# voletiv/mcvd-pytorch

Hardware: NVIDIA H100
Metric: frames/sec @100 DDPM steps, SMMNIST 64x64 (higher is better)
Workload: dtype f32 (fp16 hi/lo split on wgmma, fp32 accumulate)

## Files before the change

include/mcvd_b200.h:

```cpp
#ifndef MCVD_B200_H
#define MCVD_B200_H

#include <stdint.h>

#ifdef __cplusplus
extern "C" {
#endif

#define MCVD_ABI_VERSION 5

enum {
  MCVD_OP_NCHW_TO_NHWC = 1,
  MCVD_OP_NHWC_TO_NCHW = 2,
  MCVD_OP_TIMESTEP_EMBED = 3,
  MCVD_OP_LINEAR = 4,
  MCVD_OP_GN_PARTIAL = 5,
  MCVD_OP_GN_FINALIZE = 6,
  MCVD_OP_APPLY = 7,
  MCVD_OP_CONV_SIMT = 8,
  MCVD_OP_ATTENTION = 9,
  MCVD_OP_RESIZE_NEAREST = 10,
  MCVD_OP_DIFFUSION_UPDATE = 11,
  MCVD_OP_CONV_UMMA = 12,
  MCVD_OP_CONV_SMALLN = 13,
  MCVD_OP_COPY = 14,
  MCVD_OP_ATTENTION_UMMA = 15,
  MCVD_OP_CONV_UMMA2 = 16,
  MCVD_OP_FRAME_METRICS = 17,
  MCVD_OP_NOISE = 18,
  MCVD_OP_LPIPS_PREP = 19,
  MCVD_OP_CONV_RELU = 20,
  MCVD_OP_LPIPS_LAYER = 21,
  MCVD_OP_I3D_PREP = 22,
  MCVD_OP_CONV3D = 23,
  MCVD_OP_MAXPOOL3D = 24,
  MCVD_OP_I3D_HEAD = 25,
  MCVD_OP__COUNT
};

#define MCVD_F_ACT_IN   (1 << 0)
#define MCVD_F_ACT_OUT  (1 << 1)
#define MCVD_F_UP       (1 << 2)
#define MCVD_F_DOWN     (1 << 3)
#define MCVD_F_FILM     (1 << 4)
#define MCVD_F_CLIP     (1 << 5)
#define MCVD_F_PHILOX   (1 << 6)
#define MCVD_F_ROUND    (1 << 7)
#define MCVD_F_GAMMA    (1 << 8)
#define MCVD_F_POOL     (1 << 9)

typedef struct McvdOp {
  int32_t kind;
  int32_t flags;
  int32_t B, H, W;
  int32_t C0, C1;
  int32_t Cout;
  int32_t i0, i1, i2, i3;
  float f0, f1, f2, f3, f4, f5, f6, f7;
  const void* src0;
  const void* src1;
  const void* w;
  const void* bias;
  const void* aux0;
  const void* aux1;
  const void* aux2;
  void* dst;
  void* dst2;
  const void* src2;
  const void* src3;
  int32_t C2, C3;
  int32_t i4, i5, i6, i7;
} McvdOp;

int mcvd_abi_version(void);
int mcvd_sizeof_op(void);
const char* mcvd_last_error(void);
int mcvd_device_arch(void);

int mcvd_run_program(const McvdOp* ops, int n, void* stream);

int mcvd_validate_program(const McvdOp* ops, int n);

int mcvd_count_launches(const McvdOp* ops, int n);

long long mcvd_umma_pack_weights(const float* w_taps, int taps, int Cin, int Cout, int n_tile, int k_block,
                                 void* out, int scale_log2, void* stream);
int mcvd_umma_kblock(int C0, int C1);
int mcvd_umma2_plan(int H, int W, int ks, int C0, int C1, int C2, int C3, int n_tile, int stats);
int mcvd_umma2_plan_info(int H, int W, int ks, int C0, int C1, int C2, int C3, int n_tile, int stats, int* out);
long long mcvd_umma2_stats_bytes(int B, int H, int W, int ks, int Cout);
long long mcvd_umma2_pack_weights(const float* w_taps, int taps, int Cin, int Cout, int n_tile, int k_block,
                                  void* out, int scale_log2, int stage_off, int per_unit, void* stream);
long long mcvd_attention_scratch_bytes(int B, int T, int C);

#ifdef __cplusplus
}
#endif
#endif
```

mcvd_b200/csrc/api.cu:

```cuda
#include <stdarg.h>
#include <string.h>

#include "mcvd_common.cuh"

namespace mcvd {

static thread_local char g_err[512] = {0};

void set_error(const char* fmt, ...) {
  va_list ap;
  va_start(ap, fmt);
  vsnprintf(g_err, sizeof(g_err), fmt, ap);
  va_end(ap);
}

static int dispatch(const McvdOp& op, cudaStream_t s) {
  switch (op.kind) {
    case MCVD_OP_NCHW_TO_NHWC: return launch_nchw_to_nhwc(op, s);
    case MCVD_OP_NHWC_TO_NCHW: return launch_nhwc_to_nchw(op, s);
    case MCVD_OP_TIMESTEP_EMBED: return launch_timestep_embed(op, s);
    case MCVD_OP_LINEAR: return launch_linear(op, s);
    case MCVD_OP_GN_PARTIAL: return launch_gn_partial(op, s);
    case MCVD_OP_GN_FINALIZE: return launch_gn_finalize(op, s);
    case MCVD_OP_APPLY: return launch_apply(op, s);
    case MCVD_OP_CONV_SIMT: return launch_conv_simt(op, s);
    case MCVD_OP_ATTENTION: return launch_attention(op, s);
    case MCVD_OP_RESIZE_NEAREST: return launch_resize_nearest(op, s);
    case MCVD_OP_DIFFUSION_UPDATE: return launch_diffusion_update(op, s);
    case MCVD_OP_CONV_UMMA: return launch_conv_umma(op, s);
    case MCVD_OP_CONV_UMMA2: return launch_conv_umma2(op, s);
    case MCVD_OP_CONV_SMALLN: return launch_conv_smalln(op, s);
    case MCVD_OP_COPY: return launch_copy(op, s);
    case MCVD_OP_ATTENTION_UMMA: return launch_attention_umma(op, s);
    case MCVD_OP_FRAME_METRICS: return launch_frame_metrics(op, s);
    case MCVD_OP_NOISE: return launch_noise(op, s);
    case MCVD_OP_LPIPS_PREP: return launch_lpips_prep(op, s);
    case MCVD_OP_CONV_RELU: return launch_conv_relu(op, s);
    case MCVD_OP_LPIPS_LAYER: return launch_lpips_layer(op, s);
    case MCVD_OP_I3D_PREP: return launch_i3d_prep(op, s);
    case MCVD_OP_CONV3D: return launch_conv3d(op, s);
    case MCVD_OP_MAXPOOL3D: return launch_maxpool3d(op, s);
    case MCVD_OP_I3D_HEAD: return launch_i3d_head(op, s);
    default: break;
  }
  set_error("unknown op kind %d", op.kind);
  return -1;
}

static int validate_one(const McvdOp& op, int idx) {
  if (op.kind <= 0 || op.kind >= MCVD_OP__COUNT) {
    set_error("op %d: unknown kind %d", idx, op.kind);
    return -1;
  }
  if (op.B <= 0) {
    set_error("op %d (kind %d): batch %d", idx, op.kind, op.B);
    return -1;
  }
  const bool spatial = op.kind != MCVD_OP_TIMESTEP_EMBED && op.kind != MCVD_OP_LINEAR && op.kind != MCVD_OP_COPY;
  if (spatial && (op.H <= 0 || op.W <= 0)) {
    set_error("op %d (kind %d): spatial size %dx%d", idx, op.kind, op.H, op.W);
    return -1;
  }
  if (!op.dst || (!op.src0 && op.kind != MCVD_OP_NOISE)) {
    set_error("op %d (kind %d): null src0/dst", idx, op.kind);
    return -1;
  }
  if (op.C1 > 0 && !op.src1 && op.kind != MCVD_OP_DIFFUSION_UPDATE) {
    set_error("op %d (kind %d): C1=%d but src1 is null", idx, op.kind, op.C1);
    return -1;
  }
  auto misaligned = [](const void* p) { return p && (reinterpret_cast<uintptr_t>(p) & 15) != 0; };
  if (misaligned(op.src0) || misaligned(op.src1) || misaligned(op.dst) || misaligned(op.w) || misaligned(op.aux0) ||
      misaligned(op.aux1) || misaligned(op.aux2)) {
    set_error("op %d (kind %d): pointers must be 16-byte aligned", idx, op.kind);
    return -1;
  }
  switch (op.kind) {
    case MCVD_OP_APPLY:
      if (op.C0 % 4 || op.C1 % 4) {
        set_error("op %d APPLY: channels (%d,%d) not multiples of 4", idx, op.C0, op.C1);
        return -1;
      }
      break;
    case MCVD_OP_CONV_SIMT:
    case MCVD_OP_CONV_UMMA:
    case MCVD_OP_CONV_UMMA2:
      if (!op.w || (op.i0 != 1 && op.i0 != 3)) {
        set_error("op %d CONV: null weights or kernel size %d", idx, op.i0);
        return -1;
      }
      break;
    case MCVD_OP_ATTENTION:
    case MCVD_OP_ATTENTION_UMMA:
      if (op.i0 * op.i1 != op.C0) {
        set_error("op %d ATTENTION: heads %d x dim %d != %d", idx, op.i0, op.i1, op.C0);
        return -1;
      }
      if (op.kind == MCVD_OP_ATTENTION_UMMA && (!op.dst2 || (reinterpret_cast<uintptr_t>(op.dst2) & 15))) {
        set_error("op %d ATTENTION_UMMA: dst2 (operand-image scratch) is null or not 16-byte aligned", idx);
        return -1;
      }
      break;
    case MCVD_OP_DIFFUSION_UPDATE:
    case MCVD_OP_NOISE:
      if (op.flags & MCVD_F_GAMMA) {
        if (op.kind == MCVD_OP_DIFFUSION_UPDATE && !(op.flags & MCVD_F_PHILOX)) {
          set_error("op %d DIFFUSION_UPDATE: MCVD_F_GAMMA needs MCVD_F_PHILOX", idx);
          return -1;
        }
        if (const char* why = gamma_params_error(op)) {
          set_error("op %d (kind %d): %s", idx, op.kind, why);
          return -1;
        }
      }
      break;
    case MCVD_OP_LPIPS_PREP:
      if (!op.src1 || !op.w) {
        set_error("op %d LPIPS_PREP: null real frames or resize table", idx);
        return -1;
      }
      if (op.C0 != 1 && op.C0 != 3) {
        set_error("op %d LPIPS_PREP: %d channels per frame (1 or 3)", idx, op.C0);
        return -1;
      }
      if (op.H != 128 || op.W != 128) {
        set_error("op %d LPIPS_PREP: output side %dx%d (must be 128x128)", idx, op.H, op.W);
        return -1;
      }
      if (op.i0 < 1 || op.i1 < 1 || op.i2 < 1 || 2LL * op.B * op.i0 > 65535) {
        set_error("op %d LPIPS_PREP: %d frames of side %d, %d taps, batch %d", idx, op.i0, op.i1, op.i2, op.B);
        return -1;
      }
      break;
    case MCVD_OP_CONV_RELU:
      if (const char* why = conv_relu_error(op)) {
        set_error("op %d CONV_RELU: %s", idx, why);
        return -1;
      }
      if (misaligned(op.bias)) {
        set_error("op %d CONV_RELU: bias must be 16-byte aligned", idx);
        return -1;
      }
      break;
    case MCVD_OP_LPIPS_LAYER:
      if (!op.src1 || !op.w || op.C0 < 1) {
        set_error("op %d LPIPS_LAYER: null real features or lin weights, or %d channels", idx, op.C0);
        return -1;
      }
      break;
    case MCVD_OP_I3D_PREP:
    case MCVD_OP_CONV3D:
    case MCVD_OP_MAXPOOL3D:
    case MCVD_OP_I3D_HEAD: {
      const char* why = op.kind == MCVD_OP_I3D_PREP ? i3d_prep_error(op)
                        : op.kind == MCVD_OP_CONV3D  ? conv3d_error(op)
                        : op.kind == MCVD_OP_MAXPOOL3D ? maxpool3d_error(op)
                                                       : i3d_head_error(op);
      static const char* const names[] = {"I3D_PREP", "CONV3D", "MAXPOOL3D", "I3D_HEAD"};
      if (why) {
        set_error("op %d %s: %s", idx, names[op.kind - MCVD_OP_I3D_PREP], why);
        return -1;
      }
      if (misaligned(op.bias)) {
        set_error("op %d %s: bias must be 16-byte aligned", idx, names[op.kind - MCVD_OP_I3D_PREP]);
        return -1;
      }
      break;
    }
    default: break;
  }
  return 0;
}

}

extern "C" {

int mcvd_abi_version(void) { return MCVD_ABI_VERSION; }
int mcvd_sizeof_op(void) { return (int)sizeof(McvdOp); }
const char* mcvd_last_error(void) { return mcvd::g_err; }

int mcvd_device_arch(void) {
  int dev = 0;
  if (cudaGetDevice(&dev) != cudaSuccess) {
    cudaGetLastError();
    mcvd::set_error("no CUDA device");
    return -1;
  }
  cudaDeviceProp p;
  if (cudaGetDeviceProperties(&p, dev) != cudaSuccess) {
    cudaGetLastError();
    mcvd::set_error("cudaGetDeviceProperties failed");
    return -1;
  }
  return p.major * 10 + p.minor;
}

int mcvd_validate_program(const McvdOp* ops, int n) {
  if (!ops || n < 0) {
    mcvd::set_error("null program");
    return -1;
  }
  for (int i = 0; i < n; ++i) {
    int r = mcvd::validate_one(ops[i], i);
    if (r) return r;
  }
  return 0;
}

int mcvd_count_launches(const McvdOp* ops, int n) {
  if (!ops || n < 0) return -1;
  int total = 0;
  for (int i = 0; i < n; ++i) total += (ops[i].kind == MCVD_OP_ATTENTION_UMMA) ? 2 : 1;
  return total;
}

int mcvd_run_program(const McvdOp* ops, int n, void* stream) {
  if (!ops || n < 0) {
    mcvd::set_error("null program");
    return -1;
  }
  cudaStream_t s = reinterpret_cast<cudaStream_t>(stream);
  for (int i = 0; i < n; ++i) {
    int r = mcvd::dispatch(ops[i], s);
    if (r) {
      char tmp[400];
      strncpy(tmp, mcvd::g_err, sizeof(tmp) - 1);
      tmp[sizeof(tmp) - 1] = 0;
      mcvd::set_error("op %d (kind %d): %s", i, ops[i].kind, tmp);
      return r;
    }
  }
  return 0;
}

}
```

mcvd_b200/csrc/attention_umma.cu:

```cuda
#include "mcvd_common.cuh"
#include "umma_ptx.cuh"

namespace mcvd {

namespace {

using namespace ptx;

constexpr int QT = 128;
constexpr int ATT_THREADS = 288;
constexpr int SPLIT_THREADS = 256;

struct AttnArgs {
  const float* qkv;
  float* out;
  uint8_t* img;
  long long k_off, v_off;
  int T, C, KT, nkt, nqt, nst;
  float scale;
};

__device__ __forceinline__ void split8(const float v[8], uint4& hv, uint4& lv) {
  uint32_t hw[4], lw[4];
#pragma unroll
  for (int e = 0; e < 4; ++e) split2(v[2 * e], v[2 * e + 1], hw[e], lw[e]);
  hv = make_uint4(hw[0], hw[1], hw[2], hw[3]);
  lv = make_uint4(lw[0], lw[1], lw[2], lw[3]);
}

template <int D>
__device__ __forceinline__ void stage_rows(uint8_t* hi, uint8_t* lo, const float* src, long long stride, int rows,
                                           int valid_rows, int tid, int nthreads) {
  constexpr int U = 6;
  const int units = (D / 8) * rows;
  for (int u0 = tid; u0 < units; u0 += nthreads * U) {
    float4 va[U], vb[U];
#pragma unroll
    for (int i = 0; i < U; ++i) {
      const int u = u0 + i * nthreads;
      const int c8 = u / rows, r = u - c8 * rows;
      va[i] = vb[i] = make_float4(0.f, 0.f, 0.f, 0.f);
      if (u < units && r < valid_rows) {
        const float4* p = reinterpret_cast<const float4*>(src + (long long)r * stride + c8 * 8);
        va[i] = __ldg(p);
        vb[i] = __ldg(p + 1);
      }
    }
#pragma unroll
    for (int i = 0; i < U; ++i) {
      const int u = u0 + i * nthreads;
      if (u < units) {
        const int c8 = u / rows, r = u - c8 * rows;
        const float v[8] = {va[i].x, va[i].y, va[i].z, va[i].w, vb[i].x, vb[i].y, vb[i].z, vb[i].w};
        uint4 hv, lv;
        split8(v, hv, lv);
        const size_t off = ((size_t)c8 * rows + r) * 16;
        *reinterpret_cast<uint4*>(hi + off) = hv;
        *reinterpret_cast<uint4*>(lo + off) = lv;
      }
    }
  }
}

template <int D>
__device__ __forceinline__ void stage_v(uint8_t* vh, uint8_t* vl, const float* vsrc, long long stride, int KT, int tid,
                                        int nthreads) {
  constexpr int C4 = D / 4;
  const int vunits = (KT / 8) * C4;
  for (int u0 = tid; u0 < vunits; u0 += 2 * nthreads) {
    float4 ld[2][8];
#pragma unroll
    for (int i = 0; i < 2; ++i) {
      const int u = u0 + i * nthreads;
      const int kc = u / C4, c4 = u - kc * C4;
#pragma unroll
      for (int e = 0; e < 8; ++e)
        ld[i][e] = (u < vunits) ? __ldg(reinterpret_cast<const float4*>(vsrc + (long long)(kc * 8 + e) * stride) + c4)
                                : make_float4(0.f, 0.f, 0.f, 0.f);
    }
#pragma unroll
    for (int i = 0; i < 2; ++i) {
      const int u = u0 + i * nthreads;
      if (u < vunits) {
        const int kc = u / C4, c4 = u - kc * C4;
        const float r0[8] = {ld[i][0].x, ld[i][1].x, ld[i][2].x, ld[i][3].x, ld[i][4].x, ld[i][5].x, ld[i][6].x, ld[i][7].x};
        const float r1[8] = {ld[i][0].y, ld[i][1].y, ld[i][2].y, ld[i][3].y, ld[i][4].y, ld[i][5].y, ld[i][6].y, ld[i][7].y};
        const float r2[8] = {ld[i][0].z, ld[i][1].z, ld[i][2].z, ld[i][3].z, ld[i][4].z, ld[i][5].z, ld[i][6].z, ld[i][7].z};
        const float r3[8] = {ld[i][0].w, ld[i][1].w, ld[i][2].w, ld[i][3].w, ld[i][4].w, ld[i][5].w, ld[i][6].w, ld[i][7].w};
        uint4 hv, lv;
        const size_t off = ((size_t)kc * D + c4 * 4) * 16;
        split8(r0, hv, lv); *reinterpret_cast<uint4*>(vh + off) = hv;      *reinterpret_cast<uint4*>(vl + off) = lv;
        split8(r1, hv, lv); *reinterpret_cast<uint4*>(vh + off + 16) = hv; *reinterpret_cast<uint4*>(vl + off + 16) = lv;
        split8(r2, hv, lv); *reinterpret_cast<uint4*>(vh + off + 32) = hv; *reinterpret_cast<uint4*>(vl + off + 32) = lv;
        split8(r3, hv, lv); *reinterpret_cast<uint4*>(vh + off + 48) = hv; *reinterpret_cast<uint4*>(vl + off + 48) = lv;
      }
    }
  }
}

template <int D> __host__ __device__ constexpr int kt_max() { return D <= 96 ? 128 : (D <= 128 ? 64 : 32); }

template <int D> __host__ __device__ constexpr long long q_image_bytes() { return 2LL * (D / 8) * QT * 16; }
template <int D> __host__ __device__ inline long long kv_image_bytes(int KT) { return 2LL * (D / 8) * KT * 16; }

template <int D>
__global__ void __launch_bounds__(SPLIT_THREADS) k_attn_presplit(const AttnArgs a) {
  const int x = blockIdx.x, h = blockIdx.y, b = blockIdx.z, heads = gridDim.y;
  const int C3 = 3 * a.C, KT = a.KT;
  const float* base = a.qkv + (long long)b * a.T * C3 + h * D;
  const long long bh = (long long)b * heads + h;
  if (x < a.nqt) {
    uint8_t* dst = a.img + (bh * a.nqt + x) * q_image_bytes<D>();
    const int q0 = x * QT;
    stage_rows<D>(dst, dst + q_image_bytes<D>() / 2, base + (long long)q0 * C3, C3, QT, min(QT, a.T - q0), threadIdx.x,
                  SPLIT_THREADS);
  } else if (x < a.nqt + a.nkt) {
    const int kt = x - a.nqt;
    uint8_t* dst = a.img + a.k_off + (bh * a.nkt + kt) * kv_image_bytes<D>(KT);
    stage_rows<D>(dst, dst + kv_image_bytes<D>(KT) / 2, base + a.C + (long long)kt * KT * C3, C3, KT, KT, threadIdx.x,
                  SPLIT_THREADS);
  } else {
    const int kt = x - a.nqt - a.nkt;
    uint8_t* dst = a.img + a.v_off + (bh * a.nkt + kt) * kv_image_bytes<D>(KT);
    stage_v<D>(dst, dst + kv_image_bytes<D>(KT) / 2, base + 2 * a.C + (long long)kt * KT * C3, C3, KT, threadIdx.x,
               SPLIT_THREADS);
  }
}

template <int D, int KT>
__global__ void __launch_bounds__(ATT_THREADS, 1) k_attention_umma(const AttnArgs a) {
  extern __shared__ __align__(1024) uint8_t smem_raw[];
  constexpr int NQ = QT / 64;
  const int NST = a.nst;
  const uint32_t q_bytes = (uint32_t)q_image_bytes<D>(), kv_bytes = (uint32_t)kv_image_bytes<D>(KT);
  uint8_t* qimg = smem_raw;
  uint8_t* kimg = qimg + q_bytes;
  uint8_t* vimg = kimg + (size_t)NST * kv_bytes;
  uint64_t* bars = reinterpret_cast<uint64_t*>(vimg + (size_t)NST * kv_bytes);
  const uint32_t bar0 = smem_u32(bars);
  const uint32_t Q_FULL = bar0;
  auto K_FULL = [&](int i) { return bar0 + 8u * (1 + i); };
  auto V_FULL = [&](int i) { return bar0 + 8u * (3 + i); };
  auto K_EMPTY = [&](int i) { return bar0 + 8u * (5 + i); };
  auto V_EMPTY = [&](int i) { return bar0 + 8u * (7 + i); };

  const int tid = threadIdx.x, warp = tid >> 5, lane = tid & 31;
  const int q0 = blockIdx.x * QT, h = blockIdx.y, b = blockIdx.z;
  const long long bh = (long long)b * gridDim.y + h;

  if (tid == 0) {
    mbar_init(Q_FULL, 1);
    for (int i = 0; i < 2; ++i) {
      mbar_init(K_FULL(i), 1); mbar_init(V_FULL(i), 1);
      mbar_init(K_EMPTY(i), 4 * NQ); mbar_init(V_EMPTY(i), 4 * NQ);
    }
    fence_barrier_init();
  }
  __syncthreads();

  if (warp == 4 * NQ) {
    if (elect_one()) {
      mbar_arrive_expect_tx(Q_FULL, q_bytes);
      bulk_g2s(smem_u32(qimg), a.img + (bh * a.nqt + blockIdx.x) * q_image_bytes<D>(), q_bytes, Q_FULL);
      for (int kt = 0; kt < a.nkt; ++kt) {
        const int st = kt % NST;
        const uint32_t ph = ((kt / NST) & 1) ^ 1;
        const long long off = (bh * a.nkt + kt) * kv_image_bytes<D>(KT);
        mbar_wait(K_EMPTY(st), ph);
        mbar_arrive_expect_tx(K_FULL(st), kv_bytes);
        bulk_g2s(smem_u32(kimg + (size_t)st * kv_bytes), a.img + a.k_off + off, kv_bytes, K_FULL(st));
        mbar_wait(V_EMPTY(st), ph);
        mbar_arrive_expect_tx(V_FULL(st), kv_bytes);
        bulk_g2s(smem_u32(vimg + (size_t)st * kv_bytes), a.img + a.v_off + off, kv_bytes, V_FULL(st));
      }
    }
    __syncwarp();
    return;
  }

  const int wg = warp >> 2, wq = warp & 3;
  const int r0 = 64 * wg + 16 * wq + (lane >> 2);
  const int cq = 2 * (lane & 3);
  const uint64_t q_desc = make_desc(smem_u32(qimg) + 64u * 16u * wg, QT * 16, 128);
  const uint32_t q_lo16 = q_bytes / 32;
  const uint32_t kv_lo16 = kv_bytes / 32;
  float m[2] = {-INFINITY, -INFINITY}, l[2] = {0.f, 0.f};
  float o[D / 2];
#pragma unroll
  for (int i = 0; i < D / 2; ++i) o[i] = 0.f;
  mbar_wait(Q_FULL, 0);
  for (int kt = 0; kt < a.nkt; ++kt) {
    const int st = kt % NST;
    const uint32_t ph = (kt / NST) & 1;
    float sacc[KT / 2];
    const uint64_t k_desc = make_desc(smem_u32(kimg + (size_t)st * kv_bytes), KT * 16, 128);
    mbar_wait(K_FULL(st), ph);
    wgmma_fence();
#pragma unroll
    for (int s = 0; s < D / 16; ++s) {
      const uint64_t qh = desc_add(q_desc, 2u * s * QT), ql = desc_add(qh, q_lo16);
      const uint64_t kh = desc_add(k_desc, 2u * s * KT), kl = desc_add(kh, kv_lo16);
      wgmma_ss<KT>(sacc, qh, kh, s);
      wgmma_ss<KT>(sacc, ql, kh, 1);
      wgmma_ss<KT>(sacc, qh, kl, 1);
    }
    wgmma_commit();
    wgmma_wait<0>();
#pragma unroll
    for (int i = 0; i < KT / 2; ++i) reg_fence(sacc[i]);
    if (lane == 0) mbar_arrive(K_EMPTY(st));
    float alpha[2];
#pragma unroll
    for (int i = 0; i < 2; ++i) {
      float mx = -INFINITY;
#pragma unroll
      for (int j = 0; j < KT / 8; ++j)
        mx = fmaxf(mx, fmaxf(sacc[4 * j + 2 * i], sacc[4 * j + 2 * i + 1]));
      mx = fmaxf(mx, __shfl_xor_sync(0xffffffffu, mx, 1));
      mx = fmaxf(mx, __shfl_xor_sync(0xffffffffu, mx, 2));
      const float mn = fmaxf(m[i], mx * a.scale);
      alpha[i] = expf(m[i] - mn);
      m[i] = mn;
      float sum = 0.f;
#pragma unroll
      for (int j = 0; j < KT / 8; ++j) {
#pragma unroll
        for (int e = 0; e < 2; ++e) {
          const float p = expf(fmaf(sacc[4 * j + 2 * i + e], a.scale, -mn));
          sacc[4 * j + 2 * i + e] = p;
          sum += p;
        }
      }
      l[i] = l[i] * alpha[i] + sum;
    }
#pragma unroll
    for (int j = 0; j < D / 8; ++j) {
      o[4 * j] *= alpha[0]; o[4 * j + 1] *= alpha[0];
      o[4 * j + 2] *= alpha[1]; o[4 * j + 3] *= alpha[1];
    }
    const uint64_t v_desc = make_desc(smem_u32(vimg + (size_t)st * kv_bytes), D * 16, 128);
    mbar_wait(V_FULL(st), ph);
    uint32_t ph4[KT / 16][4], pl4[KT / 16][4];
#pragma unroll
    for (int kk = 0; kk < KT / 16; ++kk)
#pragma unroll
      for (int r = 0; r < 4; ++r) split2(sacc[8 * kk + 2 * r], sacc[8 * kk + 2 * r + 1], ph4[kk][r], pl4[kk][r]);
    wgmma_fence();
#pragma unroll
    for (int kk = 0; kk < KT / 16; ++kk) {
      const uint64_t vh = desc_add(v_desc, 2u * kk * D), vl = desc_add(vh, kv_lo16);
      wgmma_rs<D>(o, ph4[kk], vh);
      wgmma_rs<D>(o, pl4[kk], vh);
      wgmma_rs<D>(o, ph4[kk], vl);
    }
    wgmma_commit();
    wgmma_wait<0>();
#pragma unroll
    for (int i = 0; i < D / 2; ++i) reg_fence(o[i]);
    if (lane == 0) mbar_arrive(V_EMPTY(st));
  }
#pragma unroll
  for (int i = 0; i < 2; ++i) {
    l[i] += __shfl_xor_sync(0xffffffffu, l[i], 1);
    l[i] += __shfl_xor_sync(0xffffffffu, l[i], 2);
  }
#pragma unroll
  for (int i = 0; i < 2; ++i) {
    const int q = q0 + r0 + 8 * i;
    if (q >= a.T) continue;
    const float inv = 1.0f / l[i];
    float* orow = a.out + ((long long)b * a.T + q) * a.C + h * D;
#pragma unroll
    for (int j = 0; j < D / 8; ++j)
      *reinterpret_cast<float2*>(orow + 8 * j + cq) = make_float2(o[4 * j + 2 * i] * inv, o[4 * j + 2 * i + 1] * inv);
  }
}

template <int D, int KT>
int launch_dk(const AttnArgs& a, size_t smem, const McvdOp& op, cudaStream_t s) {
  cudaError_t e = cudaFuncSetAttribute(k_attention_umma<D, KT>, cudaFuncAttributeMaxDynamicSharedMemorySize, (int)smem);
  MCVD_CHECK(e == cudaSuccess, "ATTENTION_UMMA: cudaFuncSetAttribute failed: %s", cudaGetErrorString(e));
  dim3 sgrid(a.nqt + 2 * a.nkt, op.i0, op.B);
  k_attn_presplit<D><<<sgrid, SPLIT_THREADS, 0, s>>>(a);
  MCVD_CUDA_LAUNCH_CHECK("attention presplit");
  dim3 grid(a.nqt, op.i0, op.B);
  k_attention_umma<D, KT><<<grid, ATT_THREADS, smem, s>>>(a);
  MCVD_CUDA_LAUNCH_CHECK("attention_umma");
  return 0;
}

template <int D>
int launch_d(const McvdOp& op, cudaStream_t s) {
  AttnArgs a;
  a.qkv = (const float*)op.src0; a.out = (float*)op.dst;
  a.T = op.H * op.W; a.C = op.C0; a.scale = op.f0;
  a.KT = kt_max<D>();
  if (a.T < a.KT) a.KT = a.T;
  MCVD_CHECK((a.KT == 32 || a.KT == 64 || a.KT == 128) && a.T % a.KT == 0,
             "ATTENTION_UMMA: %d tokens not tileable by the key tile %d", a.T, a.KT);
  a.nkt = a.T / a.KT;
  a.nqt = cdiv(a.T, QT);
  a.img = (uint8_t*)op.dst2;
  const long long bh = (long long)op.B * op.i0;
  a.k_off = bh * a.nqt * q_image_bytes<D>();
  a.v_off = a.k_off + bh * a.nkt * kv_image_bytes<D>(a.KT);
  MCVD_CHECK(op.dst2, "ATTENTION_UMMA: dst2 (operand-image scratch, mcvd_attention_scratch_bytes) is NULL");
  MCVD_CHECK((reinterpret_cast<uintptr_t>(op.dst2) & 15) == 0, "ATTENTION_UMMA: scratch must be 16-byte aligned");
  const size_t q_bytes = (size_t)q_image_bytes<D>(), kv_bytes = (size_t)kv_image_bytes<D>(a.KT);
  a.nst = (q_bytes + 4 * kv_bytes + 128 <= 227 * 1024) ? 2 : 1;
  const size_t smem = q_bytes + 2 * a.nst * kv_bytes + 128;
  MCVD_CHECK(smem <= 227 * 1024, "ATTENTION_UMMA: %zu B of shared memory", smem);
  if (a.KT == 32) return launch_dk<D, 32>(a, smem, op, s);
  if (a.KT == 64) return launch_dk<D, (kt_max<D>() >= 64 ? 64 : 32)>(a, smem, op, s);
  return launch_dk<D, kt_max<D>()>(a, smem, op, s);
}

}

long long attention_umma_scratch_bytes(int B, int T, int C) {
  if (B <= 0 || T <= 0 || C <= 0) return 0;
  return 4LL * B * C * ((long long)cdiv(T, QT) * QT + 2LL * T);
}

int launch_attention_umma(const McvdOp& op, cudaStream_t s) {
  MCVD_CHECK(op.src0 && op.dst, "ATTENTION_UMMA: null pointer");
  MCVD_CHECK(op.i0 * op.i1 == op.C0, "ATTENTION_UMMA: heads %d x dim %d != channels %d", op.i0, op.i1, op.C0);
  switch (op.i1) {
    case 32: return launch_d<32>(op, s);
    case 48: return launch_d<48>(op, s);
    case 64: return launch_d<64>(op, s);
    case 96: return launch_d<96>(op, s);
    case 128: return launch_d<128>(op, s);
    case 192: return launch_d<192>(op, s);
    default: break;
  }
  set_error("ATTENTION_UMMA: head dim %d unsupported (32/48/64/96/128/192)", op.i1);
  return -1;
}

}

extern "C" long long mcvd_attention_scratch_bytes(int B, int T, int C) {
  return mcvd::attention_umma_scratch_bytes(B, T, C);
}
```

mcvd_b200/lib.py:

```python
from __future__ import annotations

import ctypes as C
import os
import threading

from . import build as _build

OP_NCHW_TO_NHWC = 1
OP_NHWC_TO_NCHW = 2
OP_TIMESTEP_EMBED = 3
OP_LINEAR = 4
OP_GN_PARTIAL = 5
OP_GN_FINALIZE = 6
OP_APPLY = 7
OP_CONV_SIMT = 8
OP_ATTENTION = 9
OP_RESIZE_NEAREST = 10
OP_DIFFUSION_UPDATE = 11
OP_CONV_UMMA = 12
OP_CONV_SMALLN = 13
OP_COPY = 14
OP_ATTENTION_UMMA = 15
OP_CONV_UMMA2 = 16
OP_FRAME_METRICS = 17
OP_NOISE = 18
OP_LPIPS_PREP = 19
OP_CONV_RELU = 20
OP_LPIPS_LAYER = 21
OP_I3D_PREP = 22
OP_CONV3D = 23
OP_MAXPOOL3D = 24
OP_I3D_HEAD = 25

F_ACT_IN = 1 << 0
F_ACT_OUT = 1 << 1
F_UP = 1 << 2
F_DOWN = 1 << 3
F_FILM = 1 << 4
F_CLIP = 1 << 5
F_PHILOX = 1 << 6
F_ROUND = 1 << 7
F_GAMMA = 1 << 8
F_POOL = 1 << 9

ABI_VERSION = 5

EXPORTS = ["mcvd_abi_version", "mcvd_sizeof_op", "mcvd_last_error", "mcvd_device_arch", "mcvd_run_program",
           "mcvd_validate_program", "mcvd_count_launches", "mcvd_umma_pack_weights", "mcvd_umma_kblock",
           "mcvd_attention_scratch_bytes", "mcvd_umma2_plan", "mcvd_umma2_plan_info", "mcvd_umma2_stats_bytes", "mcvd_umma2_pack_weights"]


class McvdOp(C.Structure):
    _fields_ = [
        ("kind", C.c_int32), ("flags", C.c_int32),
        ("B", C.c_int32), ("H", C.c_int32), ("W", C.c_int32),
        ("C0", C.c_int32), ("C1", C.c_int32), ("Cout", C.c_int32),
        ("i0", C.c_int32), ("i1", C.c_int32), ("i2", C.c_int32), ("i3", C.c_int32),
        ("f0", C.c_float), ("f1", C.c_float), ("f2", C.c_float), ("f3", C.c_float),
        ("f4", C.c_float), ("f5", C.c_float), ("f6", C.c_float), ("f7", C.c_float),
        ("src0", C.c_void_p), ("src1", C.c_void_p), ("w", C.c_void_p), ("bias", C.c_void_p),
        ("aux0", C.c_void_p), ("aux1", C.c_void_p), ("aux2", C.c_void_p),
        ("dst", C.c_void_p), ("dst2", C.c_void_p),
        ("src2", C.c_void_p), ("src3", C.c_void_p), ("C2", C.c_int32), ("C3", C.c_int32),
        ("i4", C.c_int32), ("i5", C.c_int32), ("i6", C.c_int32), ("i7", C.c_int32),
    ]


_lock = threading.Lock()
_lib = None


def library_path() -> str:
    return _build.LIB


def load():
    global _lib
    if _lib is not None:
        return _lib
    with _lock:
        if _lib is not None:
            return _lib
        path = _build.LIB
        if _build.needs_build():
            try:
                nvcc = _build._nvcc()
            except RuntimeError as e:
                nvcc = None
                if not os.path.exists(path):
                    raise RuntimeError(f"mcvd_b200: CUDA library missing and cannot be built: {e}") from e
                import warnings
                warnings.warn("mcvd_b200: sources are newer than the prebuilt library and nvcc is not available; "
                              "using the prebuilt library")
            if nvcc is not None:
                _build.build()
        if not os.path.exists(path):
            raise RuntimeError(f"mcvd_b200: CUDA library not found at {path}")
        lib = C.CDLL(path)
        lib.mcvd_abi_version.restype = C.c_int
        lib.mcvd_sizeof_op.restype = C.c_int
        lib.mcvd_last_error.restype = C.c_char_p
        lib.mcvd_device_arch.restype = C.c_int
        lib.mcvd_run_program.restype = C.c_int
        lib.mcvd_run_program.argtypes = [C.POINTER(McvdOp), C.c_int, C.c_void_p]
        lib.mcvd_validate_program.restype = C.c_int
        lib.mcvd_validate_program.argtypes = [C.POINTER(McvdOp), C.c_int]
        lib.mcvd_count_launches.restype = C.c_int
        lib.mcvd_count_launches.argtypes = [C.POINTER(McvdOp), C.c_int]
        lib.mcvd_umma_pack_weights.restype = C.c_longlong
        lib.mcvd_umma_pack_weights.argtypes = [C.c_void_p, C.c_int, C.c_int, C.c_int, C.c_int, C.c_int, C.c_void_p,
                                               C.c_int, C.c_void_p]
        lib.mcvd_umma_kblock.restype = C.c_int
        lib.mcvd_umma_kblock.argtypes = [C.c_int, C.c_int]
        lib.mcvd_attention_scratch_bytes.restype = C.c_longlong
        lib.mcvd_attention_scratch_bytes.argtypes = [C.c_int, C.c_int, C.c_int]
        lib.mcvd_umma2_plan.restype = C.c_int
        lib.mcvd_umma2_plan.argtypes = [C.c_int] * 9
        lib.mcvd_umma2_plan_info.restype = C.c_int
        lib.mcvd_umma2_plan_info.argtypes = [C.c_int] * 9 + [C.POINTER(C.c_int)]
        lib.mcvd_umma2_stats_bytes.restype = C.c_longlong
        lib.mcvd_umma2_stats_bytes.argtypes = [C.c_int] * 5
        lib.mcvd_umma2_pack_weights.restype = C.c_longlong
        lib.mcvd_umma2_pack_weights.argtypes = [C.c_void_p, C.c_int, C.c_int, C.c_int, C.c_int, C.c_int, C.c_void_p,
                                                C.c_int, C.c_int, C.c_int, C.c_void_p]
        if lib.mcvd_abi_version() != ABI_VERSION:
            raise RuntimeError("mcvd_b200: ABI version mismatch between the Python binding and the library")
# ... 59 lines not shown
```

mcvd_b200/program.py:

```python
from __future__ import annotations

import contextlib
import math
import os
from typing import Dict, List, Optional, Tuple

import torch

from . import arch, lib
from .lib import McvdOp

INV_SQRT2 = float(1.0 / math.sqrt(2.0))
GN_PPC = 64
GN_MIN_CHUNKS = 32


def gn_chunks(hw: int) -> int:
    return max(1, min(hw // 8, max(hw // GN_PPC, GN_MIN_CHUNKS)))


class Src:

    def __init__(self, t0, c0, t1=None, c1=0):
        self.t0, self.c0, self.t1, self.c1 = t0, c0, t1, c1

    @property
    def C(self):
        return self.c0 + self.c1


def _ptr(t) -> Optional[int]:
    return None if t is None else t.data_ptr()


def _pick_nt(cout: int) -> int:
    best = 0
    for d in range(16, 257, 16):
        if cout % d == 0:
            best = d
    return best


class Program:
    def __init__(self):
        self.keep: List[torch.Tensor] = []
        self.cond_ops: List[McvdOp] = []
        self.step_ops: List[McvdOp] = []
        self.cond_arr = None
        self.step_arr = None
        self.update_arr = None
        self.n_umma = 0
        self.n_simt = 0
        self.graph = None
        self.temb_idx: List[int] = []
        self.film_fin_idx: List[int] = []
        self.uniform_t = False

    @staticmethod
    def count_launches(ops) -> int:
        return sum(2 if o.kind == lib.OP_ATTENTION_UMMA else 1 for o in ops)

    @property
    def cond_launches(self) -> int:
        return self.count_launches(self.cond_ops)

    @property
    def step_launches(self) -> int:
        return self.count_launches(self.step_ops)


class Engine:
    def __init__(self, module, _test_backend=None):
        self.module = module
        self.spec: arch.NetSpec = module.spec
        self.device = next(module.parameters()).device
        self.backend = _test_backend
        self.lib = lib.load()
        if self.backend is None:
            if self.device.type != "cuda":
                raise RuntimeError("mcvd_b200: the module must live on a CUDA device (no CPU fallback)")
            with torch.cuda.device(self.device):
                cc = self.lib.mcvd_device_arch()
            if cc != 90:
                raise RuntimeError(f"mcvd_b200 kernels are built for sm_90a (H100) only (device reports sm_{cc}: "
                                   f"{lib.last_error()})")
        self.conv_mode = os.environ.get("MCVD_CONV", "umma").lower()
        self.split_mode = int(os.environ.get("MCVD_SPLIT", "3"))
        self.fuse_shortcut = os.environ.get("MCVD_FUSE_SC", "auto")
        self.epilogue_stats = os.environ.get("MCVD_EPISTATS", "1" if self.conv_mode == "umma2" else "0") == "1"
        self.attn_mode = os.environ.get("MCVD_ATTN", "umma").lower()
        self.use_graph = os.environ.get("MCVD_GRAPH", "1") != "0"
        self.packed: Dict[str, object] = {}
        self.packed_version = None
        self.cache_dir = os.environ.get("MCVD_WEIGHT_CACHE") or None
        self.packs_computed = 0
        self.packs_loaded = 0
        self.programs: Dict[int, Program] = {}
        self.launches_last_forward = 0

    MAX_PROGRAMS = 3

    def _version(self):
        ps = [p.detach() for p in self.module.parameters()]
        ids = tuple((p.data_ptr(), tuple(p.shape)) for p in ps)
        with torch.no_grad():
            fp = torch.stack(list(torch._foreach_norm(ps, 2)) + list(torch._foreach_norm(ps, 1))).double()
        return ids, fp

    def invalidate(self):
        self.packed_version = None

    def _sd(self, key):
        return self._params[key]

    def _cache_path(self):
        if not self.cache_dir or self.backend is not None or self.packed_version is None:
            return None
        import hashlib
        ids, fp = self.packed_version
        h = hashlib.sha256()
        h.update(repr((lib.ABI_VERSION, self.conv_mode, self.split_mode, [sh for _, sh in ids])).encode())
        h.update(fp.detach().cpu().numpy().tobytes())
        return os.path.join(self.cache_dir, f"mcvd_b200_packed_{h.hexdigest()[:32]}.pt")

    def _load_weight_cache(self):
        path = self._cache_path()
        if path is None or not os.path.exists(path):
            return
        try:
            blob = torch.load(path, map_location=self.device)
        except Exception:
            return
        for k, (t, scale) in blob.items():
            self.packed[k] = (t.to(self.device), scale)
            self._cache_loaded_keys.add(k)
        self.packs_loaded += len(blob)

    def _save_weight_cache(self):
        path = self._cache_path()
        if path is None:
            return
        blob = {k: (v[0].cpu(), v[1]) for k, v in self.packed.items()
                if isinstance(k, tuple) and len(k) > 1 and k[1] in ("umma", "umma2")}
# ... 327 lines not shown
        def spade_gb(prefix: str, C: int, H: int):
            seg = cond_resized(H)
            a = conv(cnd, prefix + "mlp_shared", Src(seg, ns.cond_ch), H, ns.spade_dim, 3,
                     prefix + "mlp_shared.0.weight", prefix + "mlp_shared.0.bias", act_out=True)
            g = conv(cnd, prefix + "mlp_gamma", Src(a, ns.spade_dim), H, C, 3, prefix + "mlp_gamma.weight",
                     prefix + "mlp_gamma.bias")
            b = conv(cnd, prefix + "mlp_beta", Src(a, ns.spade_dim), H, C, 3, prefix + "mlp_beta.weight",
                     prefix + "mlp_beta.bias")
            return g, b

        P.x_in = f32(B, ns.out_ch, S, S)
        P.cond_in = f32(B, ns.cond_ch, S, S) if ns.cond_ch > 0 else None
        P.t = f32(B)
        P.out = f32(B, ns.out_ch, S, S)
        tc_edges = self.conv_mode in ("umma", "umma2")
        in_pad = (ns.in_ch + 15) // 16 * 16 if tc_edges else ns.in_ch
        out_pad = (ns.out_ch + 15) // 16 * 16 if tc_edges else ns.out_ch
        P.noise = f32(B, ns.out_ch, S, S)
        if ns.spade:
            P.cond_nhwc = f32(B, S, S, ns.cond_ch)
            emit(cnd, lib.OP_NCHW_TO_NHWC, H=S, W=S, C0=ns.cond_ch, src0=P.cond_in, dst=P.cond_nhwc)
            xin = f32(B, S, S, in_pad)
            emit(step, lib.OP_NCHW_TO_NHWC, H=S, W=S, C0=ns.out_ch, Cout=in_pad, src0=P.x_in, dst=xin)
        else:
            xin = f32(B, S, S, in_pad)
            emit(step, lib.OP_NCHW_TO_NHWC, H=S, W=S, C0=ns.out_ch, C1=ns.cond_ch, Cout=in_pad, src0=P.x_in,
                 src1=P.cond_in, dst=xin)

        mods = ns.mods
        emb, h0, temb = f32(B, ns.nf), f32(B, ns.temb_dim), f32(B, ns.temb_dim)
        P.film = f32(B, ns.film_total)
        P.temb_idx = list(range(len(step), len(step) + 4))
        emit(step, lib.OP_TIMESTEP_EMBED, Cout=ns.nf, src0=P.t, w=self.packed["freqs"], dst=emb)
        emit(step, lib.OP_LINEAR, C0=ns.nf, Cout=ns.temb_dim, src0=emb, w=keep(sd("unet.all_modules.0.weight").float().contiguous()),
             bias=keep(sd("unet.all_modules.0.bias").float().contiguous()), dst=h0, flags=lib.F_ACT_OUT)
        emit(step, lib.OP_LINEAR, C0=ns.temb_dim, Cout=ns.temb_dim, src0=h0,
             w=keep(sd("unet.all_modules.1.weight").float().contiguous()),
             bias=keep(sd("unet.all_modules.1.bias").float().contiguous()), dst=temb, flags=lib.F_ACT_OUT)
        emit(step, lib.OP_LINEAR, C0=ns.temb_dim, Cout=ns.film_total, src0=temb, w=self.packed["film_w"],
             bias=self.packed["film_b"], dst=P.film)

        def resblock(ms: arch.ModSpec, src: Src) -> torch.Tensor:
            pre = f"unet.all_modules.{ms.idx}."
            Hin = ms.res
            H = Hin * 2 if ms.up else (Hin // 2 if ms.down else Hin)
            Cin, Cout = ms.in_ch, ms.out_ch
            eps = 1e-6 if ns.spade else 1e-5
            tab0 = norm_table(step, src, Hin, eps, film_off=ms.film_off[0])
            resample = lib.F_UP if ms.up else (lib.F_DOWN if ms.down else 0)
            sc_src = src
            if ns.spade or resample:
                g0 = b0 = None
                if ns.spade:
                    g0, b0 = spade_gb(pre + "actnorm0.Norm_0.", Cin, Hin)
                a0 = f32(B, H, H, Cin)
                xs = f32(B, H, H, Cin) if resample else None
                emit(step, lib.OP_APPLY, H=H, W=H, C0=src.c0, C1=src.c1, src0=src.t0, src1=src.t1, aux0=tab0, aux1=g0,
                     aux2=b0, dst=a0, dst2=xs, flags=lib.F_ACT_OUT | resample)
                if resample:
                    sc_src = Src(xs, Cin)
                h = conv(step, pre + "Conv_0", Src(a0, Cin), H, Cout, 3, pre + "Conv_0.weight", pre + "Conv_0.bias",
                         stats=True)
            else:
                h = conv(step, pre + "Conv_0", src, H, Cout, 3, pre + "Conv_0.weight", pre + "Conv_0.bias", tab=tab0,
                         act_in=True, stats=True)
            tab1 = norm_table(step, Src(h, Cout), H, eps, film_off=ms.film_off[1])
            shortcut = res = None
            if ms.has_shortcut:
                shortcut = (sc_src, pre + "Conv_2.weight", pre + "Conv_2.bias")
            else:
                assert src.t1 is None and src.c0 == Cout
                res = src.t0
            if ns.spade:
                g1, b1 = spade_gb(pre + "actnorm1.Norm_0.", Cout, H)
                a1 = f32(B, H, H, Cout)
                emit(step, lib.OP_APPLY, H=H, W=H, C0=Cout, src0=h, aux0=tab1, aux1=g1, aux2=b1, dst=a1,
                     flags=lib.F_ACT_OUT)
                return conv(step, pre + "Conv_1", Src(a1, Cout), H, Cout, 3, pre + "Conv_1.weight",
                            pre + "Conv_1.bias", residual=res, scale=INV_SQRT2, shortcut=shortcut, stats=True)
            return conv(step, pre + "Conv_1", Src(h, Cout), H, Cout, 3, pre + "Conv_1.weight", pre + "Conv_1.bias",
                        residual=res, scale=INV_SQRT2, tab=tab1, act_in=True, shortcut=shortcut, stats=True)

        attn_scratch = [None]

        def attnblock(ms: arch.ModSpec, x: torch.Tensor) -> torch.Tensor:
            pre = f"unet.all_modules.{ms.idx}."
            H, C = ms.res, ms.in_ch
            tab = norm_table(step, Src(x, C), H, 1e-6,
                             affine=(sd(pre + "GroupNorm_0.weight"), sd(pre + "GroupNorm_0.bias")))
            wq = torch.cat([sd(pre + f"NIN_{i}.W").float() for i in range(3)], dim=1).unsqueeze(0).contiguous()
            bq = torch.cat([sd(pre + f"NIN_{i}.b").float() for i in range(3)], dim=0).contiguous()
            qkv = conv(step, pre + "qkv", Src(x, C), H, 3 * C, 1, None, None, tab=tab, act_in=False, wcat=wq, bcat=bq)
            att = f32(B, H, H, C)
            d = C // ms.heads
            T = H * H
            kt = min(T, 128 if d <= 96 else (64 if d <= 128 else 32))
            use_tc = self.attn_mode == "umma" and d in (32, 48, 64, 96, 128, 192) and T % kt == 0 and kt in (32, 64, 128)
            if use_tc:
                need = lib.attention_scratch_bytes(B, T, C)
                if attn_scratch[0] is None or attn_scratch[0].numel() < need:
                    attn_scratch[0] = keep(torch.empty(need, device=dev, dtype=torch.uint8))
                emit(step, lib.OP_ATTENTION_UMMA, H=H, W=H, C0=C, i0=ms.heads, i1=d, f0=float(int(d) ** (-0.5)),
                     src0=qkv, dst=att, dst2=attn_scratch[0])
            else:
                emit(step, lib.OP_ATTENTION, H=H, W=H, C0=C, i0=ms.heads, i1=d, f0=float(int(d) ** (-0.5)),
                     src0=qkv, dst=att)
            return conv(step, pre + "NIN_3", Src(att, C), H, C, 1, pre + "NIN_3.W", pre + "NIN_3.b", residual=x,
                        scale=INV_SQRT2, nin=True, stats=True)

        w_first = self._conv_taps(sd("unet.all_modules.2.weight"))
        if in_pad != ns.in_ch:
            wp_ = torch.zeros(9, in_pad, ns.nf, device=dev, dtype=torch.float32)
            wp_[:, :ns.in_ch] = w_first
            w_first = wp_
        h = conv(step, "first", Src(xin, in_pad), S, ns.nf, 3, None, None, wcat=w_first,
                 bcat=sd("unet.all_modules.2.bias").float().contiguous(), stats=True)
        hs: List[Tuple[torch.Tensor, int]] = [(h, ns.nf)]
        cur, cur_c = h, ns.nf
        for ms in mods[3:-2]:
            if ms.kind == "res":
                if ms.skip_ch:
                    st, sc = hs.pop()
                    assert sc == ms.skip_ch and cur_c + sc == ms.in_ch
                    src = Src(cur, cur_c, st, sc)
                else:
                    assert cur_c == ms.in_ch
                    src = Src(cur, cur_c)
                cur, cur_c = resblock(ms, src), ms.out_ch
            elif ms.kind == "attn":
                cur = attnblock(ms, cur)
            else:
                raise AssertionError(ms.kind)
            if ms.push:
                hs.append((cur, cur_c))
        assert not hs, "skip stack not empty"

        mn, mc = mods[-2], mods[-1]
        pre = f"unet.all_modules.{mn.idx}."
        wl = self._conv_taps(sd(f"unet.all_modules.{mc.idx}.weight"))
        bl = keep(sd(f"unet.all_modules.{mc.idx}.bias").float().contiguous())
        pk = ("last", "simt")
        if pk not in self.packed:
            self.packed[pk] = self._pack_simt(wl)
        wlp, coutp = self.packed[pk]
        if ns.spade:
            tabn = norm_table(step, Src(cur, cur_c), S, 1e-6)
            gN, bN = spade_gb(pre + "Norm_0.", cur_c, S)
            an = f32(B, S, S, cur_c)
            emit(step, lib.OP_APPLY, H=S, W=S, C0=cur_c, src0=cur, aux0=tabn, aux1=gN, aux2=bN, dst=an,
                 flags=lib.F_ACT_OUT)
            last_src, tabn = an, None
        else:
            tabn = norm_table(step, Src(cur, cur_c), S, 1e-5,
                              affine=(sd(pre + "Norm_0.weight"), sd(pre + "Norm_0.bias")))
            last_src = cur
        if tc_edges:
            wl_p = torch.zeros(9, cur_c, out_pad, device=dev, dtype=torch.float32)
            wl_p[:, :, :ns.out_ch] = wl
            bl_p = torch.zeros(out_pad, device=dev, dtype=torch.float32)
            bl_p[:ns.out_ch] = bl
            P.eps_nhwc = conv(step, "last", Src(last_src, cur_c), S, out_pad, 3, None, None, tab=tabn, act_in=True,
                              wcat=wl_p, bcat=bl_p)
        elif ns.out_ch <= 16 and coutp * 9 * cur_c * 4 <= 200 * 1024:
            P.eps_nhwc = f32(B, S, S, ns.out_ch)
            emit(step, lib.OP_CONV_SMALLN, H=S, W=S, C0=cur_c, Cout=ns.out_ch, i1=coutp, src0=last_src, w=wlp, bias=bl,
                 aux0=tabn, dst=P.eps_nhwc, flags=lib.F_ACT_OUT)
        else:
            P.eps_nhwc = f32(B, S, S, ns.out_ch)
            if tabn is not None:
                an = f32(B, S, S, cur_c)
                emit(step, lib.OP_APPLY, H=S, W=S, C0=cur_c, src0=cur, aux0=tabn, dst=an, flags=lib.F_ACT_OUT)
                last_src = an
            emit(step, lib.OP_CONV_SIMT, H=S, W=S, C0=cur_c, Cout=ns.out_ch, i0=3, i1=coutp, f0=1.0, src0=last_src,
                 w=wlp, bias=bl, dst=P.eps_nhwc)
        P.eps_nhwc.zero_()
        P.n_net_ops = len(step)

        P.cond_arr = lib.make_ops(cnd) if cnd else None
        P.step_arr = lib.make_ops(step)
        o = McvdOp()
        o.kind, o.B, o.H, o.W, o.C0 = lib.OP_NHWC_TO_NCHW, B, S, S, ns.out_ch
# ... 78 lines not shown
```

Baseline: 139.2.

## Fuse attention operand hi/lo split into the UMMA kernel via producer warps

Adds a mode where the attention kernel converts Q/K/V from the fp32 qkv tensor into fp16 hi/lo operand images directly in shared memory. It uses 128 extra producer threads and mbarrier handshakes instead of a separate presplit kernel plus TMA loads from a global scratch image. This removes one launch and a global round-trip for small attention layers (at most 2 query tiles). In exchange, K/V conversion is repeated per query-tile block and the block is larger, since it always launches 384 threads.

```diff
diff --git a/include/mcvd_b200.h b/include/mcvd_b200.h
--- a/include/mcvd_b200.h
+++ b/include/mcvd_b200.h
@@ -48,6 +48,7 @@
 #define MCVD_F_ROUND    (1 << 7)
 #define MCVD_F_GAMMA    (1 << 8)
 #define MCVD_F_POOL     (1 << 9)
+#define MCVD_F_SPLIT_IN_SMEM (1 << 10)
 
 typedef struct McvdOp {
   int32_t kind;
diff --git a/mcvd_b200/csrc/api.cu b/mcvd_b200/csrc/api.cu
--- a/mcvd_b200/csrc/api.cu
+++ b/mcvd_b200/csrc/api.cu
@@ -96,7 +96,8 @@
         set_error("op %d ATTENTION: heads %d x dim %d != %d", idx, op.i0, op.i1, op.C0);
         return -1;
       }
-      if (op.kind == MCVD_OP_ATTENTION_UMMA && (!op.dst2 || (reinterpret_cast<uintptr_t>(op.dst2) & 15))) {
+      if (op.kind == MCVD_OP_ATTENTION_UMMA && !(op.flags & MCVD_F_SPLIT_IN_SMEM) &&
+          (!op.dst2 || (reinterpret_cast<uintptr_t>(op.dst2) & 15))) {
         set_error("op %d ATTENTION_UMMA: dst2 (operand-image scratch) is null or not 16-byte aligned", idx);
         return -1;
       }
@@ -211,7 +212,8 @@
 int mcvd_count_launches(const McvdOp* ops, int n) {
   if (!ops || n < 0) return -1;
   int total = 0;
-  for (int i = 0; i < n; ++i) total += (ops[i].kind == MCVD_OP_ATTENTION_UMMA) ? 2 : 1;
+  for (int i = 0; i < n; ++i)
+    total += (ops[i].kind == MCVD_OP_ATTENTION_UMMA && !(ops[i].flags & MCVD_F_SPLIT_IN_SMEM)) ? 2 : 1;
   return total;
 }
 
diff --git a/mcvd_b200/csrc/attention_umma.cu b/mcvd_b200/csrc/attention_umma.cu
--- a/mcvd_b200/csrc/attention_umma.cu
+++ b/mcvd_b200/csrc/attention_umma.cu
@@ -8,7 +8,8 @@
 using namespace ptx;
 
 constexpr int QT = 128;
-constexpr int ATT_THREADS = 288;
+constexpr int NCONV = 128;
+constexpr int ATT_THREADS = 256 + NCONV;
 constexpr int SPLIT_THREADS = 256;
 
 struct AttnArgs {
@@ -148,16 +149,42 @@
   const int q0 = blockIdx.x * QT, h = blockIdx.y, b = blockIdx.z;
   const long long bh = (long long)b * gridDim.y + h;
 
+  const uint32_t fills = a.img ? 1 : NCONV;
   if (tid == 0) {
-    mbar_init(Q_FULL, 1);
+    mbar_init(Q_FULL, fills);
     for (int i = 0; i < 2; ++i) {
-      mbar_init(K_FULL(i), 1); mbar_init(V_FULL(i), 1);
+      mbar_init(K_FULL(i), fills); mbar_init(V_FULL(i), fills);
       mbar_init(K_EMPTY(i), 4 * NQ); mbar_init(V_EMPTY(i), 4 * NQ);
     }
     fence_barrier_init();
   }
   __syncthreads();
 
+  if (warp >= 4 * NQ && !a.img) {
+    const int ct = tid - 128 * NQ;
+    const int C3 = 3 * a.C;
+    const float* base = a.qkv + (long long)b * a.T * C3 + h * D;
+    stage_rows<D>(qimg, qimg + q_bytes / 2, base + (long long)q0 * C3, C3, QT, min(QT, a.T - q0), ct, NCONV);
+    fence_proxy_async();
+    mbar_arrive(Q_FULL);
+    for (int kt = 0; kt < a.nkt; ++kt) {
+      const int st = kt % NST;
+      const uint32_t ph = ((kt / NST) & 1) ^ 1;
+      const float* kv = base + (long long)kt * KT * C3;
+      uint8_t* kd = kimg + (size_t)st * kv_bytes;
+      mbar_wait(K_EMPTY(st), ph);
+      stage_rows<D>(kd, kd + kv_bytes / 2, kv + a.C, C3, KT, KT, ct, NCONV);
+      fence_proxy_async();
+      mbar_arrive(K_FULL(st));
+      uint8_t* vd = vimg + (size_t)st * kv_bytes;
+      mbar_wait(V_EMPTY(st), ph);
+      stage_v<D>(vd, vd + kv_bytes / 2, kv + 2 * a.C, C3, KT, ct, NCONV);
+      fence_proxy_async();
+      mbar_arrive(V_FULL(st));
+    }
+    return;
+  }
+  if (warp > 4 * NQ) return;
   if (warp == 4 * NQ) {
     if (elect_one()) {
       mbar_arrive_expect_tx(Q_FULL, q_bytes);
@@ -280,9 +307,11 @@
 int launch_dk(const AttnArgs& a, size_t smem, const McvdOp& op, cudaStream_t s) {
   cudaError_t e = cudaFuncSetAttribute(k_attention_umma<D, KT>, cudaFuncAttributeMaxDynamicSharedMemorySize, (int)smem);
   MCVD_CHECK(e == cudaSuccess, "ATTENTION_UMMA: cudaFuncSetAttribute failed: %s", cudaGetErrorString(e));
-  dim3 sgrid(a.nqt + 2 * a.nkt, op.i0, op.B);
-  k_attn_presplit<D><<<sgrid, SPLIT_THREADS, 0, s>>>(a);
-  MCVD_CUDA_LAUNCH_CHECK("attention presplit");
+  if (a.img) {
+    dim3 sgrid(a.nqt + 2 * a.nkt, op.i0, op.B);
+    k_attn_presplit<D><<<sgrid, SPLIT_THREADS, 0, s>>>(a);
+    MCVD_CUDA_LAUNCH_CHECK("attention presplit");
+  }
   dim3 grid(a.nqt, op.i0, op.B);
   k_attention_umma<D, KT><<<grid, ATT_THREADS, smem, s>>>(a);
   MCVD_CUDA_LAUNCH_CHECK("attention_umma");
@@ -300,12 +329,18 @@
              "ATTENTION_UMMA: %d tokens not tileable by the key tile %d", a.T, a.KT);
   a.nkt = a.T / a.KT;
   a.nqt = cdiv(a.T, QT);
-  a.img = (uint8_t*)op.dst2;
   const long long bh = (long long)op.B * op.i0;
   a.k_off = bh * a.nqt * q_image_bytes<D>();
   a.v_off = a.k_off + bh * a.nkt * kv_image_bytes<D>(a.KT);
-  MCVD_CHECK(op.dst2, "ATTENTION_UMMA: dst2 (operand-image scratch, mcvd_attention_scratch_bytes) is NULL");
-  MCVD_CHECK((reinterpret_cast<uintptr_t>(op.dst2) & 15) == 0, "ATTENTION_UMMA: scratch must be 16-byte aligned");
+  MCVD_CHECK(a.C % 4 == 0 && (reinterpret_cast<uintptr_t>(op.src0) & 15) == 0,
+             "ATTENTION_UMMA: qkv rows must be 16-byte aligned");
+  if (op.flags & MCVD_F_SPLIT_IN_SMEM) {
+    a.img = nullptr;
+  } else {
+    a.img = (uint8_t*)op.dst2;
+    MCVD_CHECK(op.dst2, "ATTENTION_UMMA: dst2 (operand-image scratch, mcvd_attention_scratch_bytes) is NULL");
+    MCVD_CHECK((reinterpret_cast<uintptr_t>(op.dst2) & 15) == 0, "ATTENTION_UMMA: scratch must be 16-byte aligned");
+  }
   const size_t q_bytes = (size_t)q_image_bytes<D>(), kv_bytes = (size_t)kv_image_bytes<D>(a.KT);
   a.nst = (q_bytes + 4 * kv_bytes + 128 <= 227 * 1024) ? 2 : 1;
   const size_t smem = q_bytes + 2 * a.nst * kv_bytes + 128;
diff --git a/mcvd_b200/lib.py b/mcvd_b200/lib.py
--- a/mcvd_b200/lib.py
+++ b/mcvd_b200/lib.py
@@ -42,6 +42,7 @@
 F_ROUND = 1 << 7
 F_GAMMA = 1 << 8
 F_POOL = 1 << 9
+F_SPLIT_IN_SMEM = 1 << 10
 
 ABI_VERSION = 5
 
diff --git a/mcvd_b200/program.py b/mcvd_b200/program.py
--- a/mcvd_b200/program.py
+++ b/mcvd_b200/program.py
@@ -58,7 +58,7 @@
 
     @staticmethod
     def count_launches(ops) -> int:
-        return sum(2 if o.kind == lib.OP_ATTENTION_UMMA else 1 for o in ops)
+        return sum(2 if o.kind == lib.OP_ATTENTION_UMMA and not o.flags & lib.F_SPLIT_IN_SMEM else 1 for o in ops)
 
     @property
     def cond_launches(self) -> int:
@@ -552,6 +552,7 @@
                         residual=res, scale=INV_SQRT2, tab=tab1, act_in=True, shortcut=shortcut, stats=True)
 
         attn_scratch = [None]
+        split_smem_qtiles = 2
 
         def attnblock(ms: arch.ModSpec, x: torch.Tensor) -> torch.Tensor:
             pre = f"unet.all_modules.{ms.idx}."
@@ -566,7 +567,10 @@
             T = H * H
             kt = min(T, 128 if d <= 96 else (64 if d <= 128 else 32))
             use_tc = self.attn_mode == "umma" and d in (32, 48, 64, 96, 128, 192) and T % kt == 0 and kt in (32, 64, 128)
-            if use_tc:
+            if use_tc and -(-T // 128) <= split_smem_qtiles:
+                emit(step, lib.OP_ATTENTION_UMMA, H=H, W=H, C0=C, i0=ms.heads, i1=d, f0=float(int(d) ** (-0.5)),
+                     src0=qkv, dst=att, flags=lib.F_SPLIT_IN_SMEM)
+            elif use_tc:
                 need = lib.attention_scratch_bytes(B, T, C)
                 if attn_scratch[0] is None or attn_scratch[0].numel() < need:
                     attn_scratch[0] = keep(torch.empty(need, device=dev, dtype=torch.uint8))
```

New measurement: 140.1 (median of 6 runs). About the same (+0.6%).
